# gergely-flamich/compression-without-quantization

Hardware: AMD Instinct MI355X
Metric: latent blocks encoded/s at KL=16 bits (higher is better)
Workload: dtype f32

## Files before the change

compression_without_quantization_amd/build.py:

```python
import os
import subprocess
import sys

HERE = os.path.dirname(os.path.abspath(__file__))
CSRC = os.path.join(HERE, "csrc")
OUT = os.path.join(HERE, "libcwq.so")
SOURCES = ["cwq_kernels.hip", "cwq_importance.hip", "cwq_pln.hip", "cwq_partition.hip",
           "cwq_varbits.hip", "cwq_beam.hip", "cwq_backfit.hip", "cwq_capi.hip", "cwq_ac.cpp"]
HEADERS = ["cwq_math.h", "cwq_screen.h", "cwq_dispatch.h", "cwq_workspace.h", "cwq_kernels.h",
           "cwq_device.h", "cwq_debug.h", "cwq_refill.h", "cwq_imp_plan.h", "cwq_tau_guess.h",
           "cwq_beam_plan.h", "cwq_budget_plan.h"]

FLAGS = ["--offload-arch=gfx950", "-O3", "-std=c++17", "-ffp-contract=off", "-fno-fast-math",
         "-fPIC", "-shared", "-Wall", "-Wno-unused-function"]
LIBS = ["-L/opt/rocm/lib", "-lhsa-runtime64"]


def _stale():
    if not os.path.exists(OUT):
        return True
    t = os.path.getmtime(OUT)
    deps = [os.path.join(CSRC, f) for f in SOURCES + HEADERS]
    deps.append(os.path.join(HERE, "..", "include", "cwq.h"))
    deps.append(os.path.abspath(__file__))
    return any(os.path.getmtime(p) > t for p in deps if os.path.exists(p))


def build(force=False, verbose=True):
    if not force and not _stale():
        return OUT
    cmd = ["hipcc"] + FLAGS + ["-o", OUT] + [os.path.join(CSRC, s) for s in SOURCES] + LIBS
    if verbose:
        print(" ".join(cmd), flush=True)
    subprocess.check_call(cmd)
    return OUT


if __name__ == "__main__":
    build(force="--force" in sys.argv)
```

compression_without_quantization_amd/csrc/cwq_device.h:

```cpp
#pragma once
#include <hip/hip_runtime.h>
#include <stdint.h>

#include "cwq_math.h"
#include "cwq_screen.h"

namespace cwq {

static __constant__ double kLogTabConst[32] = CWQ_LOGF_TAB_INIT;

__device__ __forceinline__ void fill_logtab(double* lds) {
  if (threadIdx.x < 32) lds[threadIdx.x] = kLogTabConst[threadIdx.x];
  __syncthreads();
}

__device__ __forceinline__ float lognorm_of(float t_scale) {
  return kHalfLog2Pi + logf_full(t_scale, kLogTabConst);
}

__device__ __forceinline__ float kl_normal_normal_1(float a_loc, float a_scale, float b_loc,
                                                    float b_scale) {
  const float sa2 = a_scale * a_scale;
  const float sb2 = b_scale * b_scale;
  const float ratio = sa2 / sb2;
  const float dl = a_loc - b_loc;
  const float t1 = (dl * dl) / (2.0f * sb2);
  const float t2 = 0.5f * ((ratio - 1.0f) - logf_full(ratio, kLogTabConst));
  return t1 + t2;
}

__device__ __forceinline__ uint32_t wave_id() {
  return __builtin_amdgcn_readfirstlane(threadIdx.x >> 6);
}

__device__ __forceinline__ double wave_sum_f64(double v) {
#pragma unroll
  for (int off = 32; off >= 1; off >>= 1) v += __shfl_xor(v, off, 64);
  return v;
}
__device__ __forceinline__ double wave_max_f64(double v) {
#pragma unroll
  for (int off = 32; off >= 1; off >>= 1) {
    const double o = __shfl_xor(v, off, 64);
    v = o > v ? o : v;
  }
  return v;
}

__device__ __forceinline__ uint64_t wave_max_u64(uint64_t v) {
#pragma unroll
  for (int off = 32; off >= 1; off >>= 1) {
    uint64_t o = __shfl_xor(v, off, 64);
    v = o > v ? o : v;
  }
  return v;
}

__device__ __forceinline__ U4 philox10_dev(uint32_t c0, uint32_t c1, uint32_t c2, uint32_t c3,
                                           uint32_t k0, uint32_t k1) {
#pragma unroll
  for (int r = 0; r < 10; ++r) {
    const uint64_t p0 = (uint64_t)kPhiloxM0 * c0;
    const uint64_t p1 = (uint64_t)kPhiloxM1 * c2;
    const uint32_t n0 = __builtin_amdgcn_bitop3_b32((uint32_t)(p1 >> 32), c1, k0, 0x96);
    const uint32_t n2 = __builtin_amdgcn_bitop3_b32((uint32_t)(p0 >> 32), c3, k1, 0x96);
    c1 = (uint32_t)p1;
    c3 = (uint32_t)p0;
    c0 = n0;
    c2 = n2;
    k0 += kPhiloxW0;
    k1 += kPhiloxW1;
  }
  return U4{c0, c1, c2, c3};
}

struct PhiloxLo {
  uint32_t A, B, C, D;
};
__device__ __forceinline__ PhiloxLo philox_lo_key(const PhiloxStream& s) {
  const uint64_t p1 = (uint64_t)kPhiloxM1 * s.c2;
  const uint32_t n0 = (uint32_t)(p1 >> 32) ^ s.k0;
  const uint64_t q0 = (uint64_t)kPhiloxM0 * n0;
  PhiloxLo o;
  o.A = s.c3 ^ s.k1;
  o.B = (uint32_t)p1 ^ (s.k0 + kPhiloxW0);
  o.C = (uint32_t)(q0 >> 32) ^ (s.k1 + kPhiloxW1);
  o.D = (uint32_t)q0 ^ (s.k1 + 2u * kPhiloxW1);
  asm volatile("" : "+s"(o.A), "+s"(o.B), "+s"(o.C), "+s"(o.D));
  return o;
}
__device__ __forceinline__ U4 philox10_lo(uint32_t c0, const PhiloxLo& K, uint32_t k0,
                                          uint32_t k1) {
  const uint64_t p0 = (uint64_t)kPhiloxM0 * c0;
  const uint32_t r0n2 = (uint32_t)(p0 >> 32) ^ K.A;
  const uint64_t q1 = (uint64_t)kPhiloxM1 * r0n2;
  uint32_t x0 = (uint32_t)(q1 >> 32) ^ K.B;
  uint32_t x1 = (uint32_t)q1;
  uint32_t x2 = (uint32_t)p0 ^ K.C;
  const uint64_t s0 = (uint64_t)kPhiloxM0 * x0;
  const uint64_t s1 = (uint64_t)kPhiloxM1 * x2;
  x0 = __builtin_amdgcn_bitop3_b32((uint32_t)(s1 >> 32), x1, k0 + 2u * kPhiloxW0, 0x96);
  x2 = (uint32_t)(s0 >> 32) ^ K.D;
  x1 = (uint32_t)s1;
  uint32_t x3 = (uint32_t)s0;
  k0 += 3u * kPhiloxW0;
  k1 += 3u * kPhiloxW1;
#pragma unroll
  for (int r = 3; r < 10; ++r) {
    const uint64_t a0 = (uint64_t)kPhiloxM0 * x0;
    const uint64_t a1 = (uint64_t)kPhiloxM1 * x2;
    const uint32_t n0 = __builtin_amdgcn_bitop3_b32((uint32_t)(a1 >> 32), x1, k0, 0x96);
    const uint32_t n2 = __builtin_amdgcn_bitop3_b32((uint32_t)(a0 >> 32), x3, k1, 0x96);
    x1 = (uint32_t)a1;
    x3 = (uint32_t)a0;
    x0 = n0;
    x2 = n2;
    k0 += kPhiloxW0;
    k1 += kPhiloxW1;
  }
  return U4{x0, x1, x2, x3};
}

__device__ __forceinline__ U4 philox_block_dev(const PhiloxStream& s, uint64_t grp) {
  return philox10_dev((uint32_t)grp, (uint32_t)(grp >> 32), s.c2, s.c3, s.k0, s.k1);
}

__device__ __forceinline__ float sqrt_cr_bm(float x) {
  const float s = __builtin_amdgcn_sqrtf(x);
  const float sd = u2f(f2u(s) - 1u);
  const float su = u2f(f2u(s) + 1u);
  const float rd = __builtin_fmaf(-sd, s, x);
  const float ru = __builtin_fmaf(-su, s, x);
  const float t = (rd <= 0.0f) ? sd : s;
  return (ru > 0.0f) ? su : t;
}

__device__ __forceinline__ float bm_radius_dev(uint32_t x0, const double* logtab) {
  float u1 = uint32_to_float(x0);
  u1 = fmaxf(u1, 1.0e-7f);
  return sqrt_cr_bm(-2.0f * logf_core(u1, logtab));
}

__device__ __forceinline__ float bm_angle_dev(uint32_t x1) {
  return (float)((double)(x1 & 0x7fffffu) * 0x1.921fb54442d18p-21);
}

__device__ __forceinline__ void box_muller_dev(uint32_t x0, uint32_t x1, const double* logtab,
                                               float& f0, float& f1) {
  const float u2 = bm_radius_dev(x0, logtab);
  float s, c;
  sincosf_pos(bm_angle_dev(x1), s, c);
  f0 = s * u2;
  f1 = c * u2;
}

__device__ __forceinline__ float bm_qradius_screen(uint32_t x0) {
  const float u1 = fmaxf(uint32_to_float(x0), 1.0e-7f);
  return __builtin_amdgcn_sqrtf(-__builtin_amdgcn_logf(u1));
}
__device__ __forceinline__ void bm_sincos_screen(uint32_t x1, float& s, float& c) {
  const float V = u2f((x1 & 0x7fffffu) | 0x3f800000u);
  s = __builtin_amdgcn_sinf(V);
  c = __builtin_amdgcn_cosf(V);
}
__device__ __forceinline__ void box_muller_screen(uint32_t x0, uint32_t x1, float& f0, float& f1) {
  const float q = bm_qradius_screen(x0);
  float s, c;
  bm_sincos_screen(x1, s, c);
  f0 = s * q;
  f1 = c * q;
}

__device__ __forceinline__ F4 normal4_screen(const PhiloxStream& s, uint64_t grp) {
  const U4 x = philox_block_dev(s, grp);
  F4 z;
  box_muller_screen(x.x, x.y, z.a, z.b);
  box_muller_screen(x.z, x.w, z.c, z.d);
  return z;
}

__device__ __forceinline__ F4 normal4_screen_lo(const PhiloxStream& s, const PhiloxLo& K,
                                                uint32_t grp) {
  const U4 x = philox10_lo(grp, K, s.k0, s.k1);
  F4 z;
  box_muller_screen(x.x, x.y, z.a, z.b);
  box_muller_screen(x.z, x.w, z.c, z.d);
  return z;
}

__device__ __forceinline__ F4 normal4_dev(const PhiloxStream& s, uint64_t grp,
                                          const double* logtab) {
  const U4 x = philox_block_dev(s, grp);
  F4 z;
  box_muller_dev(x.x, x.y, logtab, z.a, z.b);
  box_muller_dev(x.z, x.w, logtab, z.c, z.d);
  return z;
}

__device__ __forceinline__ float div_rn_markstein(float a, float b, float y) {
  const float q0 = a * y;
  const float r0 = __builtin_fmaf(-b, q0, a);
  const float q1 = __builtin_fmaf(r0, y, q0);
  const float r1 = __builtin_fmaf(-b, q1, a);
  return __builtin_fmaf(r1, y, q1);
}
__device__ __forceinline__ bool markstein_ok4(float a, float b, float c, float d) {
  const float ma = __builtin_fabsf(a), mb = __builtin_fabsf(b);
  const float mc = __builtin_fabsf(c), md = __builtin_fabsf(d);
  const float hi = __builtin_fmaxf(__builtin_fmaxf(ma, mb), __builtin_fmaxf(mc, md));
  const float lo = __builtin_fminf(__builtin_fminf(ma, mb), __builtin_fminf(mc, md));
  return (hi <= 0x1p60f) & (lo >= 0x1p-60f);
}

struct BlockSpan {
  int64_t off;
  int64_t d;
};

__device__ __forceinline__ BlockSpan block_span(const int64_t* __restrict__ block_off,
                                                int64_t ud, int64_t g) {
  if (block_off == nullptr) return BlockSpan{g * ud, ud};
  int64_t a = block_off[g];
  int64_t b = block_off[g + 1];
  return BlockSpan{a, b - a};
}

__device__ __forceinline__ int32_t block_seed(int32_t seed, int64_t block_id) {
  return (int32_t)((uint32_t)seed + (uint32_t)block_id);
}

struct SeedSpec {
  int32_t seed;
  int64_t base;
  const int32_t* per_block;
  __device__ __forceinline__ int32_t of(int64_t g) const {
    return per_block ? per_block[g] : block_seed(seed, base + g);
  }
};

__device__ __forceinline__ uint32_t ord_f32(float v) {
  const uint32_t b = f2u(v);
  return (b & 0x80000000u) ? ~b : (b | 0x80000000u);
}
__device__ __forceinline__ float unord_f32(uint32_t o) {
  return u2f((o & 0x80000000u) ? (o & 0x7fffffffu) : ~o);
}
#ifndef CWQ_WAVE_MAX_ASM
#define CWQ_WAVE_MAX_ASM 1
#endif
template <int CTRL, int ROW_MASK>
__device__ __forceinline__ float dpp_max_step(float v) {
  const int ninf = (int)0xff800000u;
  const int o = __builtin_amdgcn_update_dpp(ninf, __builtin_bit_cast(int, v), CTRL, ROW_MASK, 0xf,
                                            false);
  return fmaxf(v, __builtin_bit_cast(float, o));
}
#if CWQ_WAVE_MAX_ASM
#define CWQ_DPP_MAX_STEP(v, ctl, rmask) \
  asm volatile("s_nop 1\n\tv_max_f32_dpp %0, %0, %0 " ctl " row_mask:" rmask " bank_mask:0xf" \
               : "+v"(v))
__device__ __forceinline__ float wave_max_f32(float v) {
  CWQ_DPP_MAX_STEP(v, "quad_perm:[1,0,3,2]", "0xf");
  CWQ_DPP_MAX_STEP(v, "quad_perm:[2,3,0,1]", "0xf");
  CWQ_DPP_MAX_STEP(v, "row_half_mirror", "0xf");
  CWQ_DPP_MAX_STEP(v, "row_mirror", "0xf");
  CWQ_DPP_MAX_STEP(v, "row_bcast:15", "0xa");
  CWQ_DPP_MAX_STEP(v, "row_bcast:31", "0xc");
  asm volatile("s_nop 1" : "+v"(v));
  return __builtin_bit_cast(float, __builtin_amdgcn_readlane(__builtin_bit_cast(int, v), 63));
}
#else
__device__ __forceinline__ float wave_max_f32(float v) {
  v = dpp_max_step<0xb1, 0xf>(v);
// ... 103 lines not shown
```

compression_without_quantization_amd/csrc/cwq_kernels.hip:

```cpp
#include <hip/hip_runtime.h>

#include <type_traits>
#include <stdint.h>

#include "cwq_device.h"
#include "cwq_kernels.h"
#include "cwq_refill.h"
#include "cwq_tau_guess.h"

namespace cwq {

__global__ void __launch_bounds__(256) k_prep_dims(
    const float* __restrict__ t_scale, const float* __restrict__ p_loc,
    const float* __restrict__ p_scale, int64_t n, float nst, float sdiv, float rho,
    float* __restrict__ loc_s, float* __restrict__ scale_s, float* __restrict__ lognorm,
    float* __restrict__ out_sample, unsigned long long* __restrict__ keys, int64_t nb) {
  for (int64_t g = blockIdx.x * (int64_t)blockDim.x + threadIdx.x; g < nb;
       g += (int64_t)gridDim.x * blockDim.x)
    keys[g] = 0ull;
  for (int64_t i = blockIdx.x * (int64_t)blockDim.x + threadIdx.x; i < n;
       i += (int64_t)gridDim.x * blockDim.x) {
    float ls, ss;
    shard_consts(p_loc[i], p_scale[i], nst, sdiv, rho, ls, ss);
    loc_s[i] = ls;
    scale_s[i] = ss;
    lognorm[i] = lognorm_of(t_scale[i]);
    out_sample[i] = 0.0f;
  }
}

template <int DC, bool STEP0>
__device__ __forceinline__ float eval_row(const PhiloxStream& st, uint64_t kbase, int64_t d_rt,
                                          int align_rt, const float* __restrict__ loc_s,
                                          const float* __restrict__ scale_s,
                                          const float* __restrict__ mu,
                                          const float* __restrict__ sg,
                                          const float* __restrict__ lognorm,
                                          const float* __restrict__ best,
                                          const double* logtab) {
  return eval_row_f<DC>(st, kbase, d_rt, align_rt, logtab, [&](int64_t e, float zz) -> float {
    float s = scale_s[e] * zz;
    s = loc_s[e] + s;
    const float tv = STEP0 ? s : best[e] + s;
    return log_prob(tv, mu[e], sg[e], lognorm[e]);
  });
}

template <int DC, bool STEP0>
__global__ void __launch_bounds__(256) k_encode_eval(
    const float* __restrict__ t_loc, const float* __restrict__ t_scale,
    const float* __restrict__ loc_s, const float* __restrict__ scale_s,
    const float* __restrict__ lognorm, const float* __restrict__ best,
    const int64_t* __restrict__ block_off, int64_t ud, int64_t ntiles, int64_t tiles_per_block,
    int64_t cand_per_tile, int64_t n_cand, SeedSpec sd, int32_t step,
    unsigned long long* __restrict__ keys) {
  __shared__ double logtab[32];
  __shared__ unsigned long long wkey[4];
  fill_logtab(logtab);
  const uint32_t wv = wave_id();
  const uint32_t lane = threadIdx.x & 63u;

  for (int64_t tile = blockIdx.x; tile < ntiles; tile += gridDim.x) {
    const int64_t g = tile / tiles_per_block;
    const int64_t tt = tile - g * tiles_per_block;
    const BlockSpan sp = block_span(block_off, ud, g);
    const int64_t n0 = tt * cand_per_tile;
    const int64_t n1 = (n0 + cand_per_tile < n_cand) ? n0 + cand_per_tile : n_cand;
    const PhiloxStream st =
        generate_key(step_seed(sd.of(g), step), 42);
    const int align = (int)(((uint64_t)(n0 + wv) * (uint64_t)sp.d) & 3u);

    uint64_t bestk = 0;
    for (int64_t n = n0 + 4 * (int64_t)lane + wv; n < n1; n += 256) {
      const float v = eval_row<DC, STEP0>(st, (uint64_t)n * (uint64_t)sp.d, sp.d, align,
                                          loc_s + sp.off, scale_s + sp.off, t_loc + sp.off,
                                          t_scale + sp.off, lognorm + sp.off,
                                          STEP0 ? nullptr : best + sp.off, logtab);
      const uint64_t k = argmax_key(v, (uint32_t)n);
      bestk = k > bestk ? k : bestk;
    }
    bestk = wave_max_u64(bestk);
    if (lane == 0) wkey[wv] = bestk;
    __syncthreads();
    if (threadIdx.x == 0) {
      uint64_t m = wkey[0];
      for (int i = 1; i < 4; ++i) m = wkey[i] > m ? wkey[i] : m;
      if (m) atomicMax(&keys[g], (unsigned long long)m);
    }
    __syncthreads();
  }
}

constexpr float kPruneC1 = 0x1p-14f;
#ifndef CWQ_PRUNE_MIN_WAVES
#define CWQ_PRUNE_MIN_WAVES 6
#endif
#ifndef CWQ_XCD_BALANCE
#define CWQ_XCD_BALANCE 1
#endif
#ifndef CWQ_TAU_SHARE_MASK
#define CWQ_TAU_SHARE_MASK 7u
#endif
#ifndef CWQ_CSR_TAU_SHARE_MASK
#define CWQ_CSR_TAU_SHARE_MASK 15u
#endif
#ifndef CWQ_SURVIVOR_CAP
#define CWQ_SURVIVOR_CAP 1024
#endif
#ifndef CWQ_LINKED_VISIT
#define CWQ_LINKED_VISIT 1
#endif

template <bool STEP0>
__device__ __forceinline__ float cand_diff(float z, float ls, float ss, float mu, float bb) {
  const float s = shard_sample(ls, ss, z);
  const float tv = STEP0 ? s : bb + s;
  return tv - mu;
}
__device__ __forceinline__ float lp_from_z(float z, float cc) {
  const float u = -0.5f * (z * z);
  return u - cc;
}


struct VisitRec {
  float4 sa, sb;
  int grp;
  int bk;
  int next;
  int pad;
};
static_assert(sizeof(VisitRec) == 48, "VisitRec: 48 bytes");

template <int D, bool STEP0>
__device__ __forceinline__ float score_rows_wave(
    const PhiloxStream& st, const uint32_t* rows, uint32_t cnt, const float* __restrict__ loc_s,
    const float* __restrict__ scale_s, const float* __restrict__ mu,
    const float* __restrict__ sg, const float* __restrict__ lognorm,
    const float* __restrict__ best, const double* logtab, float* buf, uint32_t lane) {
  constexpr uint32_t G = D / 4;
  const uint32_t r = lane / G, u = lane - r * G;
  if (r < cnt) {
    const F4 z = normal4_dev(st, (uint64_t)rows[r] * G + u, logtab);
#pragma unroll
    for (int t = 0; t < 4; ++t) {
      const uint32_t j = 4u * u + (uint32_t)t;
      const float zz = t == 0 ? z.a : (t == 1 ? z.b : (t == 2 ? z.c : z.d));
      float v = scale_s[j] * zz;
      v = loc_s[j] + v;
      const float tv = STEP0 ? v : best[j] + v;
      buf[r * D + j] = log_prob(tv, mu[j], sg[j], lognorm[j]);
    }
  }
  __builtin_amdgcn_fence(__ATOMIC_SEQ_CST, "wavefront");
  __builtin_amdgcn_wave_barrier();
  float acc = 0.0f;
  const uint32_t fr = lane >> 3;
  if (fr < cnt)
    for (uint32_t e = lane & 7u; e < (uint32_t)D; e += 8u) acc = acc + buf[fr * D + e];
  __builtin_amdgcn_fence(__ATOMIC_SEQ_CST, "wavefront");
  __builtin_amdgcn_wave_barrier();
  float p[8];
#pragma unroll
  for (int l = 0; l < 8; ++l) p[l] = __shfl(acc, (int)((lane & ~7u) + (uint32_t)l), 64);
  return eigen_fold8(p, 0.0f);
}

#ifdef CWQ_TILE_TIMES
constexpr int kTileTimes = 1 << 18;
__device__ unsigned long long g_tile_t0[kTileTimes], g_tile_t1[kTileTimes];
__device__ unsigned int g_tile_wg[kTileTimes];
#endif
#ifdef CWQ_PRUNE_STATS
__device__ unsigned long long g_prune_stats[72];
constexpr int kDbgBlocks = 1 << 20;
__device__ unsigned long long g_dbg_best[kDbgBlocks];
__device__ int g_seed_tau;
#endif

struct TauGuessWaveDims {
  float w, b2;
  int d;
  __device__ __forceinline__ int count() const { return d; }
  template <class F>
  __device__ __forceinline__ cwq::TauGuessSums sum(F f) const {
    cwq::TauGuessSums o = f(w, b2);
#pragma unroll
    for (int sh = 32; sh >= 1; sh >>= 1) {
      o.k += __shfl_xor(o.k, sh, 64);
      o.k1 += __shfl_xor(o.k1, sh, 64);
      o.k2 += __shfl_xor(o.k2, sh, 64);
    }
    return o;
  }
};
constexpr float kTauForceRetry = -2.0f;
__device__ __forceinline__ float tau_guess_of(float qm, float As, float Pq) {
  if (qm == kTauForceRetry) return 3.402823466e+38f;
  if (!(qm >= 0.0f)) return -__builtin_inff();
  const float tg = cwq::screen_row_lower(-qm, cwq::kScreenC2, As, Pq);
  return tg == tg ? tg : -__builtin_inff();
}

template <int D, bool STEP0, bool INTER>
__global__ void __launch_bounds__(256, CWQ_PRUNE_MIN_WAVES) k_encode_prune(
    const float* __restrict__ t_loc, const float* __restrict__ t_scale,
    const float* __restrict__ loc_s, const float* __restrict__ scale_s,
    const float* __restrict__ lognorm, const float* __restrict__ best, int64_t ntiles,
    int64_t tiles_per_block, int64_t cand_per_tile, int64_t n_cand, SeedSpec sd, int32_t step,
    int allow_screen, unsigned long long* __restrict__ keys, int64_t tail_from, int tail_div,
    uint32_t* __restrict__ tq) {
  static_assert(D % 8 == 0 && D >= 8 && D <= 64, "pruned path: D % 8 == 0, D <= 64");
  constexpr int G = D / 4;
  constexpr int NF = STEP0 ? 6 : 7;
  constexpr int RW = (64 / G) < 8 ? (64 / G) : 8;
  __shared__ double logtab[32];
  __shared__ float4 cst[G * NF];
  __shared__ VisitRec vrec[G];
  __shared__ int2 meta[G];
  __shared__ float rowbuf[4][RW * D];
  __shared__ float dscore[D];
  __shared__ float dA[D];
  __shared__ float dC[D];
  __shared__ float gscore[G];
  __shared__ int gpos[G];
  __shared__ float lowc;
  __shared__ float scr_a, scr_pq;
  __shared__ float tau_cell;
  __shared__ float tau_seed_cell;
  __shared__ float qm_cell;
  __shared__ uint32_t sq_cnt;
  __shared__ uint32_t sq_n[CWQ_SURVIVOR_CAP];
  __shared__ float sq_ub[CWQ_SURVIVOR_CAP];
  __shared__ unsigned long long wkey[4];
  __shared__ uint32_t s_next;
#ifdef CWQ_PRUNE_STATS
  __shared__ uint32_t s_ps[72];
  for (int i = threadIdx.x; i < 72; i += blockDim.x) s_ps[i] = 0u;
#endif
  fill_logtab(logtab);
  const uint32_t wv = wave_id();
  const uint32_t lane = threadIdx.x & 63u;

  constexpr bool inter = INTER;
  const int64_t nbt = INTER ? ntiles / tiles_per_block : 0;
  auto next_tile = [&](int64_t cur) -> int64_t {
    if (tq == nullptr) return cur + gridDim.x;
    __syncthreads();
    if (threadIdx.x == 0) s_next = gridDim.x + atomicAdd(tq, 1u);
    __syncthreads();
    return (int64_t)s_next;
  };
  for (int64_t tile = blockIdx.x; tile < ntiles; tile = next_tile(tile)) {
    uint32_t tid = threadIdx.x;
    asm volatile("" : "+v"(tid));
#ifdef CWQ_TILE_TIMES
    if (tid == 0 && tile < kTileTimes) {
      g_tile_t0[tile] = __builtin_amdgcn_s_memrealtime();
      const uint32_t xcc = (uint32_t)__builtin_amdgcn_s_getreg((20) | (0 << 6) | ((4 - 1) << 11));
      g_tile_wg[tile] = (xcc << 24) | (blockIdx.x & 0xffffffu);
    }
#endif
    int64_t tord = tile;
    const int64_t treg = inter ? nbt * tail_from : 0;
    if (inter && CWQ_XCD_BALANCE && tq == nullptr && tile < treg && (treg & 7) == 0 &&
        (gridDim.x & 7u) == 0)
      tord = (tile & 7) * (treg >> 3) + (tile >> 3);
    const int64_t g = inter ? tord % nbt : tile / tiles_per_block;
    const int64_t tt = inter ? tord / nbt : tile - g * tiles_per_block;
    const int64_t off = g * D;
    int64_t n0, csz;
    if (tt < tail_from) {
      n0 = tt * cand_per_tile;
      csz = cand_per_tile;
    } else {
      csz = cand_per_tile / tail_div;
      n0 = tail_from * cand_per_tile + (tt - tail_from) * csz;
    }
    const int64_t n1 = (n0 + csz < n_cand) ? n0 + csz : n_cand;
    if (n0 >= n1) continue;
    const PhiloxStream st =
        generate_key(step_seed(sd.of(g), step), 42);

    if (tid < D) {
      const int j = tid;
      const float ls = loc_s[off + j], ss = scale_s[off + j], mu = t_loc[off + j];
      const float rs = 1.0f / t_scale[off + j];
      const float m = (STEP0 ? ls : best[off + j] + ls) - mu;
      float e = 0.5f * (ss * ss + m * m) * (rs * rs);
      dscore[j] = (e == e) ? e : -1.0f;
    }
    __syncthreads();
    if (tid < G) {
      const int q = tid;
      gscore[q] = ((dscore[4 * q] + dscore[4 * q + 1]) + dscore[4 * q + 2]) + dscore[4 * q + 3];
    }
    __syncthreads();
    if (tid < G) {
      const int q = tid;
      const float sq = gscore[q];
      int r = 0;
      for (int q2 = 0; q2 < G; ++q2) {
        const float s2 = gscore[q2];
        r += (s2 > sq || (s2 == sq && q2 < q)) ? 1 : 0;
      }
      gpos[q] = r;
      meta[r].x = q;
      vrec[r].grp = q;
      vrec[r].next = r + 1 < G ? (r + 1) * (int)sizeof(VisitRec) : 0;
    }
    __syncthreads();
    int den_ok = 1, scr_ok = 1;
    if (tid < D) {
      const int j = tid, k = gpos[j >> 2], w = j & 3;
      float fj[7];
      const float sgj = t_scale[off + j];
      fj[0] = loc_s[off + j];
      fj[1] = scale_s[off + j];
      fj[2] = t_loc[off + j];
      fj[3] = sgj;
      fj[4] = lognorm[off + j];
      fj[5] = 1.0f / sgj;
      fj[6] = STEP0 ? 0.0f : best[off + j];
      float* c = reinterpret_cast<float*>(cst);
#pragma unroll
      for (int f = 0; f < NF; ++f) c[(k * NF + f) * 4 + w] = fj[f];
      den_ok = markstein_ok_den(sgj) ? 1 : 0;
      const ScreenDim o = screen_dim<STEP0>(fj[0], fj[1], fj[2], sgj, fj[4], fj[6]);
      float* sc = reinterpret_cast<float*>(&vrec[k]);
      sc[w] = o.sa;
      sc[4 + w] = o.sb;
      dA[j] = o.A;
      dC[j] = o.C;
      scr_ok = o.ok ? 1 : 0;
    }
    const bool fastdiv = __syncthreads_and(den_ok) != 0;
    const bool scr_all = __syncthreads_and(scr_ok) != 0;
    const bool screen = (allow_screen & 1) && scr_all;
    if (wv == 1u) {
      const int gmode = (allow_screen >> 1) & 3;
      float qm = cwq::kTauNoGuess;
      if (screen && gmode == 1) {
        float w = 0.0f, b2 = 0.0f;
        if (lane < (uint32_t)D) {
          const float* sc = reinterpret_cast<const float*>(&vrec[lane >> 2]);
          const float al = sc[lane & 3u] * (float)(1.0 / cwq::kSqrt2Ln2);
          const float be = sc[4u + (lane & 3u)];
          w = al * al;
          b2 = be * be;
        }
        qm = cwq::tau_guess_q(TauGuessWaveDims{w, b2, D}, n1 - n0, cwq::kTauGuessM);
      } else if (screen && gmode == 2) {
        qm = kTauForceRetry;
      }
      if (lane == 0) qm_cell = qm;
    }
    if (tid <= G + 1) {
      const int kb = tid;
      const float* c = reinterpret_cast<const float*>(cst);
      double rf = 0.0, kk = 0.0, asum = 0.0, msum = 0.0, kall = 0.0, cvis = 0.0, a2 = 0.0,
             amax = 0.0;
#pragma unroll 1
      for (int p = 0; p < D; ++p) {
        const double mj = -(double)c[((p >> 2) * NF + 4) * 4 + (p & 3)];
        const double aj = __builtin_fabs(mj);
        asum += aj;
        msum += mj;
        kall += aj + mj;
        if (p >= 4 * kb) {
          rf += mj + 0x1p-17 * aj;
        } else {
          kk += aj + mj;
          if (screen) cvis += (double)dC[(meta[p >> 2].x << 2) + (p & 3)];
        }
        if (screen && kb == G + 1) {
          const double av = (double)dA[p];
          a2 += av * av;
          amax = av > amax ? av : amax;
        }
      }
      const double marg = 0x1p-20 * (__builtin_fabs(rf) + asum) + 0x1p-126;
      const double sl = 0x1p-14 * (__builtin_fabs(msum) + asum + kall) + 0x1p-126;
      if (kb <= G) {
        const float bk = screen ? round_up_f32(msum + cvis * (1.0 + 0x1p-20) + sl)
                                : round_up_f32(rf + 0x1p-14 * kk + marg);
        if (kb >= 1) {
          meta[kb - 1].y = (int)f2u(bk);
          vrec[kb - 1].bk = (int)f2u(bk);
        }
        if (kb == G) lowc = round_up_f32(0x1p-14 * kk + marg);
      } else if (screen) {
        scr_a = screen_as(msum, sl, a2);
        scr_pq = screen_pq(amax, D);
      }
      if (kb == 0) {
        float t0 = -__builtin_inff();
        if (inter) {
          const unsigned long long kv =
              __hip_atomic_load(&keys[g], __ATOMIC_RELAXED, __HIP_MEMORY_SCOPE_AGENT);
          if ((uint32_t)(kv >> 32) > kArgmaxClampOrd) t0 = unord_f32((uint32_t)(kv >> 32));
        }
#ifdef CWQ_PRUNE_STATS
        if (g_seed_tau && g < kDbgBlocks && (g_dbg_best[g] >> 32) > kArgmaxClampOrd)
          t0 = unord_f32((uint32_t)(g_dbg_best[g] >> 32));
#endif
        tau_cell = t0;
        tau_seed_cell = t0;
        sq_cnt = 0u;
      }
    }
    __syncthreads();
    const float lc = lowc;
#ifdef CWQ_PRUNE_STATS
    const float tau_seed = tau_cell;
#endif
    const float sA = scr_a, sPq = scr_pq;

    const int64_t per_wave = (n1 - n0 + 3) / 4;
    const int64_t w0 = n0 + (int64_t)wv * per_wave;
    const int64_t w1 = (w0 + per_wave < n1) ? w0 + per_wave : n1;
    const uint32_t w0g =
        (uint32_t)__builtin_amdgcn_readfirstlane((int)((uint32_t)w0 * (uint32_t)G));
    const uint32_t wrows = w1 > w0 ? (uint32_t)(w1 - w0) : 0u;
    const uint32_t ng_end =
        (uint32_t)__builtin_amdgcn_readfirstlane((int)(wrows * (uint32_t)G));
    const uint32_t ng_stat = (uint32_t)__builtin_amdgcn_readfirstlane(
        (int)(cwq::refill_static_rows(wrows) * (uint32_t)G));
    const uint32_t ng_pool0 = (uint32_t)__builtin_amdgcn_readfirstlane(
        (int)(cwq::refill_pool_start(cwq::refill_static_rows(wrows)) * (uint32_t)G));
#ifndef CWQ_TAU_FROM_KEYS
#define CWQ_TAU_FROM_KEYS 1
#endif
    float tau = (INTER && CWQ_TAU_FROM_KEYS) ? tau_cell : -__builtin_inff();
#ifdef CWQ_PRUNE_STATS
    tau = tau_seed;
    if (tid == 0 && qm_cell >= 0.0f) atomicAdd(&g_prune_stats[50], 1ull);
#endif
    tau = max_f32_quiet(tau, tau_guess_of(qm_cell, sA, sPq));
    uint64_t bestk = 0;

    const PhiloxLo lok = philox_lo_key(st);
    auto pass = [&](auto screen_tag) {
      constexpr bool SCREEN = decltype(screen_tag)::value;
      constexpr uint32_t KS = SCREEN ? (uint32_t)sizeof(VisitRec) : 1u;
      constexpr bool LINKED = SCREEN && CWQ_LINKED_VISIT;
      uint32_t ng = lane * (uint32_t)G;
      uint32_t wnext_g = ng_pool0;
      uint32_t kp = 0;
      float s = 0.0f;
      uint32_t iter = 0;
      bool active = ng < ng_end;
      uint64_t m_act = __builtin_amdgcn_ballot_w64(active);
      while (m_act != 0ull) {
        int2 mt;
        float4 sa, sb;
        uint32_t kp_next = 0;
        if constexpr (SCREEN) {
          const char* rp = reinterpret_cast<const char*>(vrec) + kp;
          sa = *reinterpret_cast<const float4*>(rp);
          sb = *reinterpret_cast<const float4*>(rp + 16);
          const int4 lk = *reinterpret_cast<const int4*>(rp + 32);
          mt = int2{lk.x, lk.y};
          kp_next = (uint32_t)lk.z;
        } else {
          mt = meta[kp];
        }
        const uint32_t grp = (ng + (uint32_t)mt.x) + w0g;
        uint32_t pk0 = st.k0, pk1 = st.k1;
        asm volatile("" : "+s"(pk0), "+s"(pk1));
        const U4 x = philox10_lo(grp, lok, pk0, pk1);
        float z0, z1, z2, z3;
        float upper;
        if constexpr (SCREEN) {
          box_muller_screen(x.x, x.y, z0, z1);
          box_muller_screen(x.z, x.w, z2, z3);
          const float a0 = __builtin_fmaf(sa.x, z0, sb.x);
          const float a1 = __builtin_fmaf(sa.y, z1, sb.y);
          const float a2 = __builtin_fmaf(sa.z, z2, sb.z);
          const float a3 = __builtin_fmaf(sa.w, z3, sb.w);
          s = __builtin_fmaf(-a0, a0, s);
          s = __builtin_fmaf(-a1, a1, s);
          s = __builtin_fmaf(-a2, a2, s);
          s = __builtin_fmaf(-a3, a3, s);
          upper = screen_row_upper(s, kScreenC1, u2f((uint32_t)mt.y));
        } else {
          box_muller_dev(x.x, x.y, logtab, z0, z1);
          box_muller_dev(x.z, x.w, logtab, z2, z3);
          const float4* cq = cst + kp * NF;
          const float4 ls = cq[0], ss = cq[1], mu = cq[2], sg = cq[3], cc = cq[4], ry = cq[5];
          const float4 bb = STEP0 ? float4{0.f, 0.f, 0.f, 0.f} : cq[6];
          const float d0 = cand_diff<STEP0>(z0, ls.x, ss.x, mu.x, bb.x);
          const float d1 = cand_diff<STEP0>(z1, ls.y, ss.y, mu.y, bb.y);
          const float d2 = cand_diff<STEP0>(z2, ls.z, ss.z, mu.z, bb.z);
          const float d3 = cand_diff<STEP0>(z3, ls.w, ss.w, mu.w, bb.w);
          float y0 = div_rn_markstein(d0, sg.x, ry.x);
          float y1 = div_rn_markstein(d1, sg.y, ry.y);
          float y2 = div_rn_markstein(d2, sg.z, ry.z);
          float y3 = div_rn_markstein(d3, sg.w, ry.w);
          const bool ok = fastdiv & markstein_ok4(d0, d1, d2, d3);
          if (__builtin_expect(__ballot(!ok) != 0ull, 0)) {
            if (!ok) {
              y0 = d0 / sg.x;
              y1 = d1 / sg.y;
              y2 = d2 / sg.z;
              y3 = d3 / sg.w;
            }
          }
          s = s + lp_from_z(y0, cc.x);
          s = s + lp_from_z(y1, cc.y);
          s = s + lp_from_z(y2, cc.z);
          s = s + lp_from_z(y3, cc.w);
          upper = (s + __builtin_fabsf(s) * kPruneC1) + u2f((uint32_t)mt.y);
        }
        if constexpr (LINKED)
          kp = kp_next;
        else
          kp += KS;
        const bool complete = LINKED ? (kp == 0u) : (kp == KS * (uint32_t)G);
        const bool below = upper < tau;
        const bool reach = SCREEN ? !below : (upper >= tau);
#ifdef CWQ_PRUNE_STATS
        const bool prune = !complete && below;
        const uint32_t k = (LINKED && complete) ? (uint32_t)G : kp / KS;
#endif
        const bool done = complete || below || !active;
        const uint64_t m_cpl = __builtin_amdgcn_ballot_w64(complete);
        const uint64_t m_below = __builtin_amdgcn_fcmpf(upper, tau, 4 );
        uint64_t m = m_cpl | m_below | (__builtin_amdgcn_read_exec() & ~m_act);
        uint64_t m_keep =
            m_cpl & m_act &
            (SCREEN ? ~m_below : (uint64_t)__builtin_amdgcn_fcmpf(upper, tau, 3 ));
        asm volatile("" : "+s"(m), "+s"(m_keep));
        if (__builtin_expect(m_keep != 0ull, 0)) {
          const bool keep = complete && active && reach;
          float lower;
          if constexpr (SCREEN)
            lower = screen_row_lower(s, kScreenC2, sA, sPq);
          else
            lower = (s - __builtin_fabsf(s) * kPruneC1) - lc;
          tau = tau_raise_wave(tau, keep, lower);
          if (__builtin_expect(keep && upper >= tau, 0)) {
            uint32_t ngc = ng;
            asm volatile("" : "+v"(ngc));
            const uint32_t n = (w0g + ngc) / (uint32_t)G;
#ifdef CWQ_PRUNE_STATS
            atomicAdd(&s_ps[66], 1u);
#endif
            const uint32_t slot = atomicAdd(&sq_cnt, 1u);
            if (slot < CWQ_SURVIVOR_CAP) {
              sq_n[slot] = (uint32_t)n;
              sq_ub[slot] = upper;
            } else {
#ifdef CWQ_PRUNE_STATS
              atomicAdd(&g_prune_stats[69], 1ull);
#endif
              const float v = eval_row<D, STEP0>(st, (uint64_t)n * D, D, 0, loc_s + off,
                                                 scale_s + off, t_loc + off, t_scale + off,
                                                 lognorm + off, STEP0 ? nullptr : best + off, logtab);
              const uint64_t kv = argmax_key(v, (uint32_t)n);
              bestk = kv > bestk ? kv : bestk;
            }
          }
        }
#ifdef CWQ_PRUNE_STATS
        if (active && (complete || prune)) atomicAdd(&s_ps[k], 1u);
        if (active && complete) atomicAdd(&s_ps[65], 1u);
#endif
        if (done) {
          asm volatile("" : "+v"(ng));
          ng += 64u * (uint32_t)G;
          kp = 0;
          s = 0.0f;
        }
        if (((++iter) & CWQ_TAU_SHARE_MASK) == 0u) tau = tau_share_wave(&tau_cell, tau);
        const uint64_t m_pool = m & __builtin_amdgcn_uicmp(ng, ng_stat, 35 );
        if (m_pool != 0ull) {
#ifdef CWQ_PRUNE_STATS
          if (lane == 0) atomicAdd(&s_ps[70], 1u);
#endif
          const uint32_t rank = __builtin_amdgcn_mbcnt_hi(
              (uint32_t)(m_pool >> 32), __builtin_amdgcn_mbcnt_lo((uint32_t)m_pool, 0u));
          if (done && ng >= ng_stat) ng = wnext_g + rank * (uint32_t)G;
          wnext_g += (uint32_t)__builtin_popcountll(m_pool) * (uint32_t)G;
          wnext_g = wnext_g < ng_end ? wnext_g : ng_end;
          active = ng < ng_end;
          m_act = __builtin_amdgcn_ballot_w64(active);
        }
#ifdef CWQ_PRUNE_STATS
        if (lane == 0) atomicAdd(&s_ps[71], 1u);
#endif
      }
    };
#ifdef CWQ_PRUNE_STATS
    if (screen && tid == 0) atomicAdd(&g_prune_stats[67], 1ull);
#endif
    float tau_final;
    if (screen) {
      for (;;) {
        pass(std::true_type{});
        tau_share_wave(&tau_cell, tau);
        __syncthreads();
        tau_final = tau_cell;
        const float tg = tau_guess_of(qm_cell, sA, sPq);
        const float seed = INTER ? tau_seed_cell : -__builtin_inff();
        const bool held = tau_final > tg || seed >= tg;
        if (__builtin_amdgcn_readfirstlane(held ? 1 : 0) != 0) break;
        __syncthreads();
        if (tid == 0) {
          tau_cell = seed;
          sq_cnt = 0u;
          qm_cell = cwq::kTauNoGuess;
#ifdef CWQ_PRUNE_STATS
          atomicAdd(&g_prune_stats[51], 1ull);
#endif
        }
        __syncthreads();
        tau = (INTER && CWQ_TAU_FROM_KEYS) ? seed : -__builtin_inff();
      }
    } else {
      pass(std::false_type{});
      tau_share_wave(&tau_cell, tau);
      __syncthreads();
      tau_final = tau_cell;
    }
    const uint32_t nsurv = sq_cnt < CWQ_SURVIVOR_CAP ? sq_cnt : CWQ_SURVIVOR_CAP;
    const uint32_t nsurv_u = (uint32_t)__builtin_amdgcn_readfirstlane((int)nsurv);
    const uint32_t sl = tid & 63u;
    for (uint32_t c0 = wv * 64u; c0 < nsurv_u; c0 += 256u) {
      const uint32_t i = c0 + sl;
      const bool q = i < nsurv_u && sq_ub[i] >= tau_final;
      const uint32_t nn = i < nsurv_u ? sq_n[i] : 0u;
      const uint64_t qm = __builtin_amdgcn_ballot_w64(q);
      if (qm == 0ull) continue;
#ifdef CWQ_PRUNE_STATS
      if (q) atomicAdd(&g_prune_stats[68], 1ull);
#endif
      const uint32_t qr = __builtin_amdgcn_mbcnt_hi((uint32_t)(qm >> 32),
                                                    __builtin_amdgcn_mbcnt_lo((uint32_t)qm, 0u));
      __builtin_amdgcn_fence(__ATOMIC_SEQ_CST, "wavefront");
      __builtin_amdgcn_wave_barrier();
      if (q) sq_n[c0 + qr] = nn;
      __builtin_amdgcn_fence(__ATOMIC_SEQ_CST, "wavefront");
      __builtin_amdgcn_wave_barrier();
      const uint32_t qn = (uint32_t)__builtin_popcountll(qm);
      for (uint32_t b = 0; b < qn; b += (uint32_t)RW) {
        const uint32_t cnt = qn - b < (uint32_t)RW ? qn - b : (uint32_t)RW;
        const float v = score_rows_wave<D, STEP0>(
            st, sq_n + c0 + b, cnt, loc_s + off, scale_s + off, t_loc + off, t_scale + off,
            lognorm + off, STEP0 ? nullptr : best + off, logtab, rowbuf[wv], sl);
        if ((sl & 7u) == 0u && (sl >> 3) < cnt) {
          const uint64_t kv = argmax_key(v, sq_n[c0 + b + (sl >> 3)]);
          bestk = kv > bestk ? kv : bestk;
        }
      }
    }

    bestk = wave_max_u64(bestk);
    if (lane == 0) wkey[wv] = bestk;
    __syncthreads();
    if (tid == 0) {
      uint64_t mk = wkey[0];
      for (int i = 1; i < 4; ++i) mk = wkey[i] > mk ? wkey[i] : mk;
      if (mk) atomicMax(&keys[g], (unsigned long long)mk);
#ifdef CWQ_PRUNE_STATS
      if (!g_seed_tau && g < kDbgBlocks) g_dbg_best[g] = mk;
#endif
#ifdef CWQ_TILE_TIMES
      if (tile < kTileTimes) g_tile_t1[tile] = __builtin_amdgcn_s_memrealtime();
#endif
    }
#ifdef CWQ_PRUNE_STATS
    if (tid < 72) {
      if (s_ps[tid]) atomicAdd(&g_prune_stats[tid], (unsigned long long)s_ps[tid]);
      s_ps[tid] = 0u;
    }
#endif
    __syncthreads();
  }
}

__device__ __forceinline__ double block_sum_d(double v, double* red) {
  red[threadIdx.x] = v;
  __syncthreads();
  for (int w = 128; w > 0; w >>= 1) {
    if ((int)threadIdx.x < w) red[threadIdx.x] += red[threadIdx.x + w];
    __syncthreads();
  }
  const double r = red[0];
  __syncthreads();
  return r;
}

__host__ __device__ __forceinline__ int64_t csr_cls_stride(int64_t d) { return (d + 6) / 4 + 1; }
constexpr int64_t kCsrSortUnits = 2048;

template <bool STEP0>
__global__ void __launch_bounds__(256) k_csr_prep(
    const float* __restrict__ t_loc, const float* __restrict__ t_scale,
    const float* __restrict__ loc_s, const float* __restrict__ scale_s,
    const float* __restrict__ lognorm, const float* __restrict__ best,
    const int64_t* __restrict__ block_off, int64_t ud, int64_t nb, float2* __restrict__ sab,
    float* __restrict__ cdim, float* __restrict__ bpre, uint32_t* __restrict__ ordu,
    float4* __restrict__ grp, uint32_t* __restrict__ gtau, float4* __restrict__ abp,
    int64_t lds_dims, int64_t coop_min_d) {
  __shared__ double red[5][4];
  __shared__ double wscan[4];
  __shared__ double ucs[256];
  __shared__ unsigned long long skey[kCsrSortUnits];
  const int tid = threadIdx.x;
  const int lane = tid & 63, wv = tid >> 6;
  const bool lead = blockIdx.y == 0;
  for (int64_t g = blockIdx.x; g < nb; g += gridDim.x) {
    const BlockSpan sp = block_span(block_off, ud, g);
    const int64_t off = sp.off, d = sp.d;
    ScreenSums u;
    float2* sabg = sab + off + 8 * g + 4;
    float* cg = cdim + off;
    if (lead && tid < 8) {
      if (tid < 4) sabg[tid - 4] = float2{0.f, 0.f};
      sabg[d + tid] = float2{0.f, 0.f};
    }
    for (int64_t j = tid; j < d; j += 256) {
      const ScreenDim o =
          screen_dim<STEP0>(loc_s[off + j], scale_s[off + j], t_loc[off + j], t_scale[off + j],
                            lognorm[off + j], STEP0 ? 0.0f : best[off + j]);
      sabg[j] = float2{o.sa, o.sb};
      cg[j] = o.C;
      u.add(o);
    }
    u.sm = wave_sum_f64(u.sm);
    u.sa = wave_sum_f64(u.sa);
    u.sk = wave_sum_f64(u.sk);
    u.s2 = wave_sum_f64(u.s2);
    u.mx = wave_max_f64(u.mx);
    if (lane == 0) {
      red[0][wv] = u.sm;
      red[1][wv] = u.sa;
      red[2][wv] = u.sk;
      red[3][wv] = u.s2;
// ... 2680 lines not shown
```

Measured before the change: 3.765 million.

## Fold Philox round-0 addend into visit records and borrow refill lanes

The first Philox multiply is precomputed as an addend stored in per-wave visit records, so the hot loop computes the round-0 product as a single multiply-add instead of adding the group offset before multiplying. The pool refill logic is rewritten in inline assembly, with lanes starting from a borrowed offset and exec-masked updates, and a range-skip fast path that avoids the ballot recompute. Visit records are replicated per wave, which increases LDS use. The inline-asm exec manipulation is fragile.

```diff
diff --git a/compression_without_quantization_amd/build.py b/compression_without_quantization_amd/build.py
--- a/compression_without_quantization_amd/build.py
+++ b/compression_without_quantization_amd/build.py
@@ -9,7 +9,7 @@
            "cwq_varbits.hip", "cwq_beam.hip", "cwq_backfit.hip", "cwq_capi.hip", "cwq_ac.cpp"]
 HEADERS = ["cwq_math.h", "cwq_screen.h", "cwq_dispatch.h", "cwq_workspace.h", "cwq_kernels.h",
            "cwq_device.h", "cwq_debug.h", "cwq_refill.h", "cwq_imp_plan.h", "cwq_tau_guess.h",
-           "cwq_beam_plan.h", "cwq_budget_plan.h"]
+           "cwq_beam_plan.h", "cwq_budget_plan.h", "cwq_philox_lo.h"]
 
 FLAGS = ["--offload-arch=gfx950", "-O3", "-std=c++17", "-ffp-contract=off", "-fno-fast-math",
          "-fPIC", "-shared", "-Wall", "-Wno-unused-function"]
diff --git a/compression_without_quantization_amd/csrc/cwq_device.h b/compression_without_quantization_amd/csrc/cwq_device.h
--- a/compression_without_quantization_amd/csrc/cwq_device.h
+++ b/compression_without_quantization_amd/csrc/cwq_device.h
@@ -3,6 +3,7 @@
 #include <stdint.h>
 
 #include "cwq_math.h"
+#include "cwq_philox_lo.h"
 #include "cwq_screen.h"
 
 namespace cwq {
@@ -74,51 +75,10 @@
   return U4{c0, c1, c2, c3};
 }
 
-struct PhiloxLo {
-  uint32_t A, B, C, D;
-};
 __device__ __forceinline__ PhiloxLo philox_lo_key(const PhiloxStream& s) {
-  const uint64_t p1 = (uint64_t)kPhiloxM1 * s.c2;
-  const uint32_t n0 = (uint32_t)(p1 >> 32) ^ s.k0;
-  const uint64_t q0 = (uint64_t)kPhiloxM0 * n0;
-  PhiloxLo o;
-  o.A = s.c3 ^ s.k1;
-  o.B = (uint32_t)p1 ^ (s.k0 + kPhiloxW0);
-  o.C = (uint32_t)(q0 >> 32) ^ (s.k1 + kPhiloxW1);
-  o.D = (uint32_t)q0 ^ (s.k1 + 2u * kPhiloxW1);
+  PhiloxLo o = philox_lo_words(s);
   asm volatile("" : "+s"(o.A), "+s"(o.B), "+s"(o.C), "+s"(o.D));
   return o;
-}
-__device__ __forceinline__ U4 philox10_lo(uint32_t c0, const PhiloxLo& K, uint32_t k0,
-                                          uint32_t k1) {
-  const uint64_t p0 = (uint64_t)kPhiloxM0 * c0;
-  const uint32_t r0n2 = (uint32_t)(p0 >> 32) ^ K.A;
-  const uint64_t q1 = (uint64_t)kPhiloxM1 * r0n2;
-  uint32_t x0 = (uint32_t)(q1 >> 32) ^ K.B;
-  uint32_t x1 = (uint32_t)q1;
-  uint32_t x2 = (uint32_t)p0 ^ K.C;
-  const uint64_t s0 = (uint64_t)kPhiloxM0 * x0;
-  const uint64_t s1 = (uint64_t)kPhiloxM1 * x2;
-  x0 = __builtin_amdgcn_bitop3_b32((uint32_t)(s1 >> 32), x1, k0 + 2u * kPhiloxW0, 0x96);
-  x2 = (uint32_t)(s0 >> 32) ^ K.D;
-  x1 = (uint32_t)s1;
-  uint32_t x3 = (uint32_t)s0;
-  k0 += 3u * kPhiloxW0;
-  k1 += 3u * kPhiloxW1;
-#pragma unroll
-  for (int r = 3; r < 10; ++r) {
-    const uint64_t a0 = (uint64_t)kPhiloxM0 * x0;
-    const uint64_t a1 = (uint64_t)kPhiloxM1 * x2;
-    const uint32_t n0 = __builtin_amdgcn_bitop3_b32((uint32_t)(a1 >> 32), x1, k0, 0x96);
-    const uint32_t n2 = __builtin_amdgcn_bitop3_b32((uint32_t)(a0 >> 32), x3, k1, 0x96);
-    x1 = (uint32_t)a1;
-    x3 = (uint32_t)a0;
-    x0 = n0;
-    x2 = n2;
-    k0 += kPhiloxW0;
-    k1 += kPhiloxW1;
-  }
-  return U4{x0, x1, x2, x3};
 }
 
 __device__ __forceinline__ U4 philox_block_dev(const PhiloxStream& s, uint64_t grp) {
diff --git a/compression_without_quantization_amd/csrc/cwq_kernels.hip b/compression_without_quantization_amd/csrc/cwq_kernels.hip
--- a/compression_without_quantization_amd/csrc/cwq_kernels.hip
+++ b/compression_without_quantization_amd/csrc/cwq_kernels.hip
@@ -110,6 +110,15 @@
 #ifndef CWQ_LINKED_VISIT
 #define CWQ_LINKED_VISIT 1
 #endif
+#ifndef CWQ_FOLD_ROUND0
+#define CWQ_FOLD_ROUND0 1
+#endif
+#ifndef CWQ_BORROW_REFILL
+#define CWQ_BORROW_REFILL 1
+#endif
+#ifndef CWQ_POOL_RANGE_SKIP
+#define CWQ_POOL_RANGE_SKIP 1
+#endif
 
 template <bool STEP0>
 __device__ __forceinline__ float cand_diff(float z, float ls, float ss, float mu, float bb) {
@@ -125,10 +134,9 @@
 
 struct VisitRec {
   float4 sa, sb;
-  int grp;
+  uint32_t add[2];
   int bk;
   int next;
-  int pad;
 };
 static_assert(sizeof(VisitRec) == 48, "VisitRec: 48 bytes");
 
@@ -194,6 +202,11 @@
     return o;
   }
 };
+__device__ __forceinline__ uint64_t sgpr_pair_uniform(uint64_t v) {
+  const uint32_t lo = (uint32_t)__builtin_amdgcn_readfirstlane((int)(uint32_t)v);
+  const uint32_t hi = (uint32_t)__builtin_amdgcn_readfirstlane((int)(uint32_t)(v >> 32));
+  return ((uint64_t)hi << 32) | lo;
+}
 constexpr float kTauForceRetry = -2.0f;
 __device__ __forceinline__ float tau_guess_of(float qm, float As, float Pq) {
   if (qm == kTauForceRetry) return 3.402823466e+38f;
@@ -216,7 +229,9 @@
   constexpr int RW = (64 / G) < 8 ? (64 / G) : 8;
   __shared__ double logtab[32];
   __shared__ float4 cst[G * NF];
-  __shared__ VisitRec vrec[G];
+  constexpr int NREC = CWQ_FOLD_ROUND0 ? 4 : 1;
+  __shared__ VisitRec vrec[NREC * G];
+  __shared__ uint32_t w0g_cell[4];
   __shared__ int2 meta[G];
   __shared__ float rowbuf[4][RW * D];
   __shared__ float dscore[D];
@@ -306,8 +321,16 @@
       }
       gpos[q] = r;
       meta[r].x = q;
-      vrec[r].grp = q;
-      vrec[r].next = r + 1 < G ? (r + 1) * (int)sizeof(VisitRec) : 0;
+#pragma unroll
+      for (int w = 0; w < NREC; ++w) {
+        const uint32_t wg = (uint32_t)(n0 + (int64_t)w * ((n1 - n0 + 3) / 4)) * (uint32_t)G;
+        const uint64_t add =
+            CWQ_FOLD_ROUND0 ? cwq::philox_round0_addend(wg + (uint32_t)q) : (uint64_t)q;
+        VisitRec& v = vrec[w * G + r];
+        v.add[0] = (uint32_t)add;
+        v.add[1] = (uint32_t)(add >> 32);
+        v.next = r + 1 < G ? (w * G + r + 1) * (int)sizeof(VisitRec) : 0;
+      }
     }
     __syncthreads();
     int den_ok = 1, scr_ok = 1;
@@ -327,9 +350,12 @@
       for (int f = 0; f < NF; ++f) c[(k * NF + f) * 4 + w] = fj[f];
       den_ok = markstein_ok_den(sgj) ? 1 : 0;
       const ScreenDim o = screen_dim<STEP0>(fj[0], fj[1], fj[2], sgj, fj[4], fj[6]);
-      float* sc = reinterpret_cast<float*>(&vrec[k]);
-      sc[w] = o.sa;
-      sc[4 + w] = o.sb;
+#pragma unroll
+      for (int c = 0; c < NREC; ++c) {
+        float* sc = reinterpret_cast<float*>(&vrec[c * G + k]);
+        sc[w] = o.sa;
+        sc[4 + w] = o.sb;
+      }
       dA[j] = o.A;
       dC[j] = o.C;
       scr_ok = o.ok ? 1 : 0;
@@ -386,7 +412,8 @@
                                 : round_up_f32(rf + 0x1p-14 * kk + marg);
         if (kb >= 1) {
           meta[kb - 1].y = (int)f2u(bk);
-          vrec[kb - 1].bk = (int)f2u(bk);
+#pragma unroll
+          for (int c = 0; c < NREC; ++c) vrec[c * G + kb - 1].bk = (int)f2u(bk);
         }
         if (kb == G) lowc = round_up_f32(0x1p-14 * kk + marg);
       } else if (screen) {
@@ -421,6 +448,7 @@
     const int64_t w1 = (w0 + per_wave < n1) ? w0 + per_wave : n1;
     const uint32_t w0g =
         (uint32_t)__builtin_amdgcn_readfirstlane((int)((uint32_t)w0 * (uint32_t)G));
+    if (lane == 0) w0g_cell[wv] = w0g;
     const uint32_t wrows = w1 > w0 ? (uint32_t)(w1 - w0) : 0u;
     const uint32_t ng_end =
         (uint32_t)__builtin_amdgcn_readfirstlane((int)(wrows * (uint32_t)G));
@@ -428,6 +456,9 @@
         (int)(cwq::refill_static_rows(wrows) * (uint32_t)G));
     const uint32_t ng_pool0 = (uint32_t)__builtin_amdgcn_readfirstlane(
         (int)(cwq::refill_pool_start(cwq::refill_static_rows(wrows)) * (uint32_t)G));
+    const uint32_t ng_first =
+        (CWQ_BORROW_REFILL && ng_stat != 0u) ? ng_stat - 64u * (uint32_t)G : 0u;
+    const uint32_t kbase = CWQ_FOLD_ROUND0 ? wv * (uint32_t)(G * sizeof(VisitRec)) : 0u;
 #ifndef CWQ_TAU_FROM_KEYS
 #define CWQ_TAU_FROM_KEYS 1
 #endif
@@ -444,31 +475,45 @@
       constexpr bool SCREEN = decltype(screen_tag)::value;
       constexpr uint32_t KS = SCREEN ? (uint32_t)sizeof(VisitRec) : 1u;
       constexpr bool LINKED = SCREEN && CWQ_LINKED_VISIT;
-      uint32_t ng = lane * (uint32_t)G;
+      uint32_t ng = ng_first + lane * (uint32_t)G;
       uint32_t wnext_g = ng_pool0;
-      uint32_t kp = 0;
+      uint64_t left;
+      asm volatile("s_cmp_eq_u32 %1, 0\n\ts_cselect_b64 %0, -1, 0" : "=s"(left) : "s"(ng_stat) : "scc");
+      const uint32_t kb = SCREEN ? kbase : 0u;
+      uint32_t kp = kb;
       float s = 0.0f;
       uint32_t iter = 0;
+      uint32_t w0g_x = 0u;
+      if constexpr (!SCREEN || !CWQ_FOLD_ROUND0) w0g_x = w0g;
       bool active = ng < ng_end;
       uint64_t m_act = __builtin_amdgcn_ballot_w64(active);
       while (m_act != 0ull) {
         int2 mt;
         float4 sa, sb;
         uint32_t kp_next = 0;
+        uint64_t p0;
         if constexpr (SCREEN) {
           const char* rp = reinterpret_cast<const char*>(vrec) + kp;
           sa = *reinterpret_cast<const float4*>(rp);
           sb = *reinterpret_cast<const float4*>(rp + 16);
-          const int4 lk = *reinterpret_cast<const int4*>(rp + 32);
-          mt = int2{lk.x, lk.y};
-          kp_next = (uint32_t)lk.z;
+          typedef int v4i __attribute__((ext_vector_type(4)));
+          v4i lk = *reinterpret_cast<const v4i*>(rp + 32);
+          if constexpr (CWQ_FOLD_ROUND0) asm volatile("" : "+v"(lk));
+          mt = int2{lk.x, lk.z};
+          kp_next = (uint32_t)lk.w;
+          if constexpr (CWQ_FOLD_ROUND0) {
+            p0 = cwq::philox_round0_product(
+                ng, (uint64_t)(uint32_t)lk.x | ((uint64_t)(uint32_t)lk.y << 32));
+          } else {
+            p0 = (uint64_t)kPhiloxM0 * ((ng + (uint32_t)mt.x) + w0g_x);
+          }
         } else {
           mt = meta[kp];
-        }
-        const uint32_t grp = (ng + (uint32_t)mt.x) + w0g;
+          p0 = (uint64_t)kPhiloxM0 * ((ng + (uint32_t)mt.x) + w0g_x);
+        }
         uint32_t pk0 = st.k0, pk1 = st.k1;
         asm volatile("" : "+s"(pk0), "+s"(pk1));
-        const U4 x = philox10_lo(grp, lok, pk0, pk1);
+        const U4 x = philox10_lo_p0(p0, lok, pk0, pk1);
         float z0, z1, z2, z3;
         float upper;
         if constexpr (SCREEN) {
@@ -516,12 +561,12 @@
           kp = kp_next;
         else
           kp += KS;
-        const bool complete = LINKED ? (kp == 0u) : (kp == KS * (uint32_t)G);
+        const bool complete = LINKED ? (kp == 0u) : (kp == kb + KS * (uint32_t)G);
         const bool below = upper < tau;
         const bool reach = SCREEN ? !below : (upper >= tau);
 #ifdef CWQ_PRUNE_STATS
         const bool prune = !complete && below;
-        const uint32_t k = (LINKED && complete) ? (uint32_t)G : kp / KS;
+        const uint32_t k = (LINKED && complete) ? (uint32_t)G : (kp - kb) / KS;
 #endif
         const bool done = complete || below || !active;
         const uint64_t m_cpl = __builtin_amdgcn_ballot_w64(complete);
@@ -532,7 +577,8 @@
             (SCREEN ? ~m_below : (uint64_t)__builtin_amdgcn_fcmpf(upper, tau, 3 ));
         asm volatile("" : "+s"(m), "+s"(m_keep));
         if (__builtin_expect(m_keep != 0ull, 0)) {
-          const bool keep = complete && active && reach;
+          const bool keep = CWQ_BORROW_REFILL ? ((m_keep >> lane) & 1ull) != 0ull
+                                              : (complete && active && reach);
           float lower;
           if constexpr (SCREEN)
             lower = screen_row_lower(s, kScreenC2, sA, sPq);
@@ -542,7 +588,8 @@
           if (__builtin_expect(keep && upper >= tau, 0)) {
             uint32_t ngc = ng;
             asm volatile("" : "+v"(ngc));
-            const uint32_t n = (w0g + ngc) / (uint32_t)G;
+            const uint32_t n =
+                (*const_cast<const volatile uint32_t*>(&w0g_cell[wv]) + ngc) / (uint32_t)G;
 #ifdef CWQ_PRUNE_STATS
             atomicAdd(&s_ps[66], 1u);
 #endif
@@ -563,28 +610,73 @@
           }
         }
 #ifdef CWQ_PRUNE_STATS
-        if (active && (complete || prune)) atomicAdd(&s_ps[k], 1u);
-        if (active && complete) atomicAdd(&s_ps[65], 1u);
-#endif
-        if (done) {
-          asm volatile("" : "+v"(ng));
-          ng += 64u * (uint32_t)G;
-          kp = 0;
-          s = 0.0f;
+        const bool act_l = ((m_act >> lane) & 1ull) != 0ull;
+        if (act_l && (complete || prune)) atomicAdd(&s_ps[k], 1u);
+        if (act_l && complete) atomicAdd(&s_ps[65], 1u);
+#endif
+        uint64_t m_pool;
+        if constexpr (CWQ_BORROW_REFILL) {
+          asm volatile(
+              "s_mov_b64 exec, %[m]\n\t"
+              "v_subrev_co_u32 %[ng], vcc, %[c], %[ng]\n\t"
+              "v_mov_b32 %[kp], %[kb]\n\t"
+              "v_mov_b32 %[s], 0\n\t"
+              "s_mov_b64 exec, -1\n\t"
+              "s_and_b64 %[mp], vcc, %[m]\n\t"
+              "s_or_b64 %[left], %[left], %[mp]\n\t"
+              "s_and_b64 %[mp], %[left], %[m]"
+              : [ng] "+v"(ng), [kp] "+v"(kp), [s] "+v"(s), [mp] "=&s"(m_pool),
+                [left] "+s"(left)
+              : [m] "s"(m), [c] "n"(64 * G), [kb] "s"(kb)
+              : "vcc", "scc");
+          left = sgpr_pair_uniform(left);
+          m_pool = sgpr_pair_uniform(m_pool);
+        } else {
+          if (done) {
+            asm volatile("" : "+v"(ng));
+            ng += 64u * (uint32_t)G;
+            kp = kb;
+            s = 0.0f;
+          }
+          m_pool = 0ull;
         }
         if (((++iter) & CWQ_TAU_SHARE_MASK) == 0u) tau = tau_share_wave(&tau_cell, tau);
-        const uint64_t m_pool = m & __builtin_amdgcn_uicmp(ng, ng_stat, 35 );
-        if (m_pool != 0ull) {
+        if constexpr (CWQ_BORROW_REFILL) {
+          if (m_pool != 0ull) {
 #ifdef CWQ_PRUNE_STATS
-          if (lane == 0) atomicAdd(&s_ps[70], 1u);
-#endif
-          const uint32_t rank = __builtin_amdgcn_mbcnt_hi(
-              (uint32_t)(m_pool >> 32), __builtin_amdgcn_mbcnt_lo((uint32_t)m_pool, 0u));
-          if (done && ng >= ng_stat) ng = wnext_g + rank * (uint32_t)G;
-          wnext_g += (uint32_t)__builtin_popcountll(m_pool) * (uint32_t)G;
-          wnext_g = wnext_g < ng_end ? wnext_g : ng_end;
-          active = ng < ng_end;
-          m_act = __builtin_amdgcn_ballot_w64(active);
+            if (lane == 0) atomicAdd(&s_ps[70], 1u);
+#endif
+            const uint32_t rank = __builtin_amdgcn_mbcnt_hi(
+                (uint32_t)(m_pool >> 32), __builtin_amdgcn_mbcnt_lo((uint32_t)m_pool, 0u));
+            asm volatile(
+                "s_mov_b64 exec, %[mp]\n\t"
+                "v_mad_u32_u24 %[ng], %[rank], %[g], %[wn]\n\t"
+                "s_mov_b64 exec, -1"
+                : [ng] "+v"(ng)
+                : [mp] "s"(m_pool), [rank] "v"(rank), [g] "n"(G), [wn] "s"(wnext_g));
+            const uint32_t want = wnext_g + (uint32_t)__builtin_popcountll(m_pool) * (uint32_t)G;
+            if (CWQ_POOL_RANGE_SKIP && want <= ng_end) {
+              wnext_g = want;
+              m_act |= m_pool;
+            } else {
+              wnext_g = want < ng_end ? want : ng_end;
+              m_act = __builtin_amdgcn_uicmp(ng, ng_end, 36 );
+            }
+          }
+        } else {
+          m_pool = m & __builtin_amdgcn_uicmp(ng, ng_stat, 35 );
+          if (m_pool != 0ull) {
+#ifdef CWQ_PRUNE_STATS
+            if (lane == 0) atomicAdd(&s_ps[70], 1u);
+#endif
+            const uint32_t rank = __builtin_amdgcn_mbcnt_hi(
+                (uint32_t)(m_pool >> 32), __builtin_amdgcn_mbcnt_lo((uint32_t)m_pool, 0u));
+            if (done && ng >= ng_stat) ng = wnext_g + rank * (uint32_t)G;
+            wnext_g += (uint32_t)__builtin_popcountll(m_pool) * (uint32_t)G;
+            wnext_g = wnext_g < ng_end ? wnext_g : ng_end;
+            active = ng < ng_end;
+            m_act = __builtin_amdgcn_ballot_w64(active);
+          }
         }
 #ifdef CWQ_PRUNE_STATS
         if (lane == 0) atomicAdd(&s_ps[71], 1u);
diff --git a/compression_without_quantization_amd/csrc/cwq_philox_lo.h b/compression_without_quantization_amd/csrc/cwq_philox_lo.h
--- /dev/null
+++ b/compression_without_quantization_amd/csrc/cwq_philox_lo.h
@@ -0,0 +1,69 @@
+#pragma once
+#include <stdint.h>
+
+#include "cwq_math.h"
+
+#if defined(__HIP_DEVICE_COMPILE__)
+#define CWQ_XOR3(a, b, c) __builtin_amdgcn_bitop3_b32((a), (b), (c), 0x96)
+#else
+#define CWQ_XOR3(a, b, c) ((a) ^ (b) ^ (c))
+#endif
+
+namespace cwq {
+
+struct PhiloxLo {
+  uint32_t A, B, C, D;
+};
+
+CWQ_HD PhiloxLo philox_lo_words(const PhiloxStream& s) {
+  const uint64_t p1 = (uint64_t)kPhiloxM1 * s.c2;
+  const uint32_t n0 = (uint32_t)(p1 >> 32) ^ s.k0;
+  const uint64_t q0 = (uint64_t)kPhiloxM0 * n0;
+  PhiloxLo o;
+  o.A = s.c3 ^ s.k1;
+  o.B = (uint32_t)p1 ^ (s.k0 + kPhiloxW0);
+  o.C = (uint32_t)(q0 >> 32) ^ (s.k1 + kPhiloxW1);
+  o.D = (uint32_t)q0 ^ (s.k1 + 2u * kPhiloxW1);
+  return o;
+}
+
+CWQ_HD uint64_t philox_round0_addend(uint32_t g) { return (uint64_t)kPhiloxM0 * g; }
+CWQ_HD uint64_t philox_round0_product(uint32_t X, uint64_t addend) {
+  return (uint64_t)kPhiloxM0 * X + addend;
+}
+
+CWQ_HD U4 philox10_lo_p0(uint64_t p0, const PhiloxLo& K, uint32_t k0, uint32_t k1) {
+  const uint32_t r0n2 = (uint32_t)(p0 >> 32) ^ K.A;
+  const uint64_t q1 = (uint64_t)kPhiloxM1 * r0n2;
+  uint32_t x0 = (uint32_t)(q1 >> 32) ^ K.B;
+  uint32_t x1 = (uint32_t)q1;
+  uint32_t x2 = (uint32_t)p0 ^ K.C;
+  const uint64_t s0 = (uint64_t)kPhiloxM0 * x0;
+  const uint64_t s1 = (uint64_t)kPhiloxM1 * x2;
+  x0 = CWQ_XOR3((uint32_t)(s1 >> 32), x1, k0 + 2u * kPhiloxW0);
+  x2 = (uint32_t)(s0 >> 32) ^ K.D;
+  x1 = (uint32_t)s1;
+  uint32_t x3 = (uint32_t)s0;
+  k0 += 3u * kPhiloxW0;
+  k1 += 3u * kPhiloxW1;
+#pragma unroll
+  for (int r = 3; r < 10; ++r) {
+    const uint64_t a0 = (uint64_t)kPhiloxM0 * x0;
+    const uint64_t a1 = (uint64_t)kPhiloxM1 * x2;
+    const uint32_t n0 = CWQ_XOR3((uint32_t)(a1 >> 32), x1, k0);
+    const uint32_t n2 = CWQ_XOR3((uint32_t)(a0 >> 32), x3, k1);
+    x1 = (uint32_t)a1;
+    x3 = (uint32_t)a0;
+    x0 = n0;
+    x2 = n2;
+    k0 += kPhiloxW0;
+    k1 += kPhiloxW1;
+  }
+  return U4{x0, x1, x2, x3};
+}
+
+CWQ_HD U4 philox10_lo(uint32_t c0, const PhiloxLo& K, uint32_t k0, uint32_t k1) {
+  return philox10_lo_p0((uint64_t)kPhiloxM0 * c0, K, k0, k1);
+}
+
+}
```

Result: faster. 3.847 million (median of 6 runs) (+2.2%).
